# rcallahan/smalt

Hardware: AMD Instinct MI355X
Metric: mapped reads/sec (1Mx150bp vs 3Gbp ref) (higher is better)
Workload: dtype f16

## Files before the change

include/smaltgpu.h:

```cpp
#ifndef SMALTGPU_H
#define SMALTGPU_H
#include <stddef.h>
#include <stdint.h>

#ifdef __cplusplus
extern "C" {
#endif

enum {
  SMALTGPU_OK = 0,
  SMALTGPU_ENODEV = -1,
  SMALTGPU_EFILE = -2,
  SMALTGPU_EARG = -3,
  SMALTGPU_ENOMEM = -4,
  SMALTGPU_ECAP = -5,
  SMALTGPU_EINTERNAL = -6,
  SMALTGPU_ESCORE = -8,
  SMALTGPU_ECPLX = -9
};
#define SMALTGPU_IS_READ_ERROR(rv) ((rv) == SMALTGPU_ECAP || (rv) == SMALTGPU_EINTERNAL || (rv) == SMALTGPU_ESCORE || (rv) == SMALTGPU_ECPLX)

enum {
  SMALTGPU_FLG_CMPLXW = 0x01,
  SMALTGPU_FLG_BEST = 0x02,
// ... 239 lines not shown
typedef struct smaltgpu_inshist smaltgpu_inshist;
int smaltgpu_sample_interval(uint64_t npairs, int every);
int smaltgpu_inshist_from_sample(smaltgpu_inshist **out, const int32_t *sample, uint64_t n);
int smaltgpu_inshist_read(smaltgpu_inshist **out, const char *path);
void smaltgpu_inshist_free(smaltgpu_inshist *h);
enum { SMALTGPU_HIST_SAMPLED = 0, SMALTGPU_HIST_SMOOTHED = 1, SMALTGPU_HIST_SECTION = 2 };
int smaltgpu_inshist_text(smaltgpu_inshist *h, int what, int width, const char **text, uint64_t *len);
int smaltgpu_inshist_bounds(const smaltgpu_inshist *h, int32_t *lo, int32_t *hi, int32_t *nbins, uint64_t *total);
int smaltgpu_inshist_count(const smaltgpu_inshist *h, int32_t insert_size, int smoothed, int32_t *count, int32_t *cumulative);
int smaltgpu_report_set_inshist(smaltgpu_report *rp, const smaltgpu_inshist *h);
int smaltgpu_report_pair_inserts(const smaltgpu_report *rp, const int32_t **insert_size, const uint8_t **known, uint32_t *npairs);

int smaltgpu_index_seqnames(const smaltgpu_index *ix, const char *const **names, const uint64_t **sop, int64_t *nseq);

int smaltgpu_timers(const smaltgpu_mapper *m, double *ms, uint64_t *work, int n);
const char *smaltgpu_timer_name(int i);

int smaltgpu_set_debug(smaltgpu_mapper *m, int level);
long smaltgpu_dump_read(smaltgpu_mapper *m, uint32_t i, const char *name, char *buf, size_t bufsiz);

int smaltgpu_sw_full_batch(smaltgpu_mapper *m, const uint8_t *qcodes, const uint32_t *q_off, const uint8_t *rcodes,
                           const uint32_t *r_off, uint32_t ntask, const smaltgpu_params *par, int32_t *scores, int packed16);

int smaltgpu_rank_sort_batch(smaltgpu_mapper *m, const uint32_t *keys, const uint32_t *off, uint32_t narr, int nneed, int in_lds,
                             uint32_t *out_keys, uint32_t *out_idx);

const char *smaltgpu_last_error(void);
int smaltgpu_device_count(void);

#ifdef __cplusplus
}
#endif
#endif
```

smalt_amd/api.py:

```python
from __future__ import annotations

import ctypes as C
import os
from typing import List, Optional, Sequence

HERE = os.path.dirname(os.path.abspath(__file__))
LIBPATH = os.path.join(HERE, "libsmaltgpu.so")

FLG_CMPLXW, FLG_BEST, FLG_SEQBYSEQ, FLG_NOSHRTINFO, FLG_SENSITIVE = 0x01, 0x02, 0x10, 0x20, 0x80
ECAP, EINTERNAL, ESCORE, ECPLX = -5, -6, -8, -9


class SmaltGpuError(RuntimeError):
    def __init__(self, code, msg):
        super().__init__("smaltgpu error %d: %s" % (code, msg))
        self.code = code


class IndexDesc(C.Structure):
    _fields_ = [("k", C.c_int32), ("s", C.c_int32), ("typ", C.c_int32), ("nbits_key", C.c_int32), ("nbits_lo", C.c_int32),
                ("npos", C.c_uint32), ("nwords", C.c_uint32), ("idx", C.c_void_p), ("pos", C.c_void_p),
                ("wordidx", C.c_void_p), ("posidx", C.c_void_p), ("nseq", C.c_int64), ("sop", C.c_void_p),
                ("packed", C.c_void_p), ("on_device", C.c_int32)]

# ... 137 lines not shown
        L.smaltgpu_report_emit.argtypes = [C.c_void_p, C.POINTER(PostOut), C.POINTER(BatchOut), C.POINTER(ReadsView), C.POINTER(C.c_char_p), C.c_int64,
                                           C.POINTER(ReportOpts), C.c_int, C.POINTER(C.c_void_p), C.POINTER(C.c_uint64)]
        L.smaltgpu_pairs_create.restype = C.c_void_p
        L.smaltgpu_pairs_free.argtypes = [C.c_void_p]
        L.smaltgpu_map_pairs.argtypes = [C.c_void_p, C.c_void_p, C.c_void_p, C.c_void_p, C.c_void_p, C.c_void_p, C.c_void_p, C.c_uint32, C.POINTER(Params),
                                         C.POINTER(PairOpts), C.c_void_p]
        L.smaltgpu_pairs_timers.argtypes = [C.c_void_p, C.POINTER(C.c_double), C.POINTER(C.c_uint64)]
        L.smaltgpu_map_pairs_resident.argtypes = [C.c_void_p, C.POINTER(ResidentReads), C.c_void_p, C.c_void_p, C.c_void_p, C.c_void_p, C.c_uint32, C.POINTER(Params),
                                                  C.POINTER(PairOpts), C.c_void_p]
        L.smaltgpu_pairs_info.argtypes = [C.c_void_p, C.POINTER(C.c_uint32), C.POINTER(C.POINTER(PairInfo)), C.POINTER(C.c_uint64), C.POINTER(C.c_double)]
        L.smaltgpu_report_emit_pairs.argtypes = [C.c_void_p, C.c_void_p, C.POINTER(ReadsView), C.POINTER(ReadsView), C.POINTER(C.c_char_p), C.c_int64,
                                                 C.POINTER(ReportOpts), C.POINTER(PairOpts), C.c_int, C.POINTER(C.c_void_p), C.POINTER(C.c_uint64)]
        L.smaltgpu_index_seqnames.argtypes = [C.c_void_p, C.POINTER(C.POINTER(C.c_char_p)), C.POINTER(C.POINTER(C.c_uint64)), C.POINTER(C.c_int64)]
        L.smaltgpu_map_batch_device.argtypes = [C.c_void_p, C.c_void_p, C.c_void_p, C.c_void_p, C.c_uint32, C.c_uint64,
                                                C.POINTER(Params)]
        L.smaltgpu_fetch_results.argtypes = [C.c_void_p, C.POINTER(BatchOut)]
        L.smaltgpu_synchronize.argtypes = [C.c_void_p]
        L.smaltgpu_timers.argtypes = [C.c_void_p, C.POINTER(C.c_double), C.POINTER(C.c_uint64), C.c_int]
        L.smaltgpu_set_debug.argtypes = [C.c_void_p, C.c_int]
        L.smaltgpu_dump_read.restype = C.c_long
        L.smaltgpu_dump_read.argtypes = [C.c_void_p, C.c_uint32, C.c_char_p, C.c_char_p, C.c_size_t]
        L.smaltgpu_sw_full_batch.argtypes = [C.c_void_p, C.c_char_p, C.POINTER(C.c_uint32), C.c_char_p,
                                             C.POINTER(C.c_uint32), C.c_uint32, C.POINTER(Params), C.POINTER(C.c_int32), C.c_int]
        L.smaltgpu_rank_sort_batch.argtypes = [C.c_void_p, C.c_void_p, C.c_void_p, C.c_uint32, C.c_int, C.c_int, C.c_void_p, C.c_void_p]
        L.smaltgpu_sample_interval.argtypes = [C.c_uint64, C.c_int]
        L.smaltgpu_inshist_from_sample.argtypes = [C.POINTER(C.c_void_p), C.POINTER(C.c_int32), C.c_uint64]
        L.smaltgpu_inshist_read.argtypes = [C.POINTER(C.c_void_p), C.c_char_p]
        L.smaltgpu_inshist_free.argtypes = [C.c_void_p]
        L.smaltgpu_inshist_text.argtypes = [C.c_void_p, C.c_int, C.c_int, C.POINTER(C.c_void_p), C.POINTER(C.c_uint64)]
        L.smaltgpu_inshist_bounds.argtypes = [C.c_void_p, C.POINTER(C.c_int32), C.POINTER(C.c_int32), C.POINTER(C.c_int32), C.POINTER(C.c_uint64)]
        L.smaltgpu_inshist_count.argtypes = [C.c_void_p, C.c_int32, C.c_int, C.POINTER(C.c_int32), C.POINTER(C.c_int32)]
        L.smaltgpu_report_set_inshist.argtypes = [C.c_void_p, C.c_void_p]
        L.smaltgpu_report_pair_inserts.argtypes = [C.c_void_p, C.POINTER(C.POINTER(C.c_int32)), C.POINTER(C.POINTER(C.c_uint8)), C.POINTER(C.c_uint32)]
        _lib = L
    return _lib


def _check(rv):
    if rv != 0:
        raise SmaltGpuError(rv, lib().smaltgpu_last_error().decode())


def device_count() -> int:
    return lib().smaltgpu_device_count()


# ... 334 lines not shown
```

smalt_amd/csrc/smaltgpu.cpp:

```cpp
#include <hip/hip_runtime.h>
#include <math.h>
#include <stdarg.h>
#include <stdio.h>
#include <stdlib.h>
#include <string.h>
#include <mutex>
#include <string>
#include <thread>
#include <vector>
#include "../../include/smaltgpu.h"
#include "smg_dump.hpp"
#include "smg_indexfile.hpp"
#include "smg_indexbuild.h"
#include "smg_fasta.hpp"
#include "smg_kernels.h"

using namespace smg;

static thread_local std::string g_err;
static int fail(int code, const char *fmt, ...) {
  char buf[512];
  va_list ap;
  va_start(ap, fmt);
  vsnprintf(buf, sizeof(buf), fmt, ap);
// ... 1192 lines not shown
  uint32_t qmaxlen = 0;
  for (uint32_t t = 0; t < ntask; t++) { uint32_t l = q_off[t + 1] - q_off[t]; if (l > qmaxlen) qmaxlen = l; }
  int rv = 0;
  if (dalloc(&dq, q_off[ntask] + 16) || dalloc(&dr, r_off[ntask] + 16) || dalloc(&dqo, (size_t)ntask + 1) || dalloc(&dro, (size_t)ntask + 1) || dalloc(&dsc, ntask)) rv = SMALTGPU_ENOMEM;
  if (!rv) {
    (void)hipMemcpy(dq, qcodes, q_off[ntask], hipMemcpyHostToDevice);
    (void)hipMemcpy(dr, rcodes, r_off[ntask], hipMemcpyHostToDevice);
    (void)hipMemcpy(dqo, q_off, ((size_t)ntask + 1) * 4, hipMemcpyHostToDevice);
    (void)hipMemcpy(dro, r_off, ((size_t)ntask + 1) * 4, hipMemcpyHostToDevice);
    uint32_t rmaxlen = 0;
    for (uint32_t t = 0; t < ntask; t++) { uint32_t l = r_off[t + 1] - r_off[t]; if (l > rmaxlen) rmaxlen = l; }
    int lr;
    if (!packed16 && (qmaxlen > 512 || rmaxlen > (uint32_t)SW_FULL_WMAX))
      lr = launch_sw_strip_raw(m->stream, dq, dqo, dr, dro, ntask, to_par(par), dsc, m->strip_bnd, m->strip_win, m->wincap, m->strip_grid);
    else lr = launch_sw_full_raw(m->stream, dq, dqo, dr, dro, ntask, to_par(par), dsc, qmaxlen, packed16);
    if (lr) rv = fail(SMALTGPU_EARG, lr == -2 ? "scores do not fit the packed 16-bit kernel" : "query longer than the register-tiled kernel supports");
    else if (hipStreamSynchronize(m->stream) != hipSuccess) rv = fail(SMALTGPU_ENODEV, "kernel failed");
    else (void)hipMemcpy(scores, dsc, (size_t)ntask * 4, hipMemcpyDeviceToHost);
  }
  (void)hipFree(dq); (void)hipFree(dr); (void)hipFree(dqo); (void)hipFree(dro); (void)hipFree(dsc);
  return rv;
}

extern "C" int smaltgpu_rank_sort_batch(smaltgpu_mapper *m, const uint32_t *keys, const uint32_t *off, uint32_t narr, int nneed, int in_lds,
                                         uint32_t *out_keys, uint32_t *out_idx) {
  if (!m || !keys || !off || !out_keys || !out_idx) return fail(SMALTGPU_EARG, "null argument");
  HIPCHK(hipSetDevice(m->device));
  const size_t tot = off[narr];
  for (uint32_t t = 0; t < narr; t++) if (off[t + 1] < off[t] || off[t + 1] - off[t] > (1u << 22)) return fail(SMALTGPU_EARG, "bad array offsets");
  for (size_t i = 0; i < tot; i++) if (keys[i] >= 1024u) return fail(SMALTGPU_EARG, "key out of range");
  uint32_t *dk = nullptr, *doff = nullptr, *dkv = nullptr, *dok = nullptr, *doi = nullptr;
  int rv = 0;
  if (dalloc(&dk, tot + 1) || dalloc(&doff, (size_t)narr + 1) || dalloc(&dkv, tot + 1) || dalloc(&dok, tot + 1) || dalloc(&doi, tot + 1)) rv = SMALTGPU_ENOMEM;
  if (!rv) {
    (void)hipMemcpy(dk, keys, tot * 4, hipMemcpyHostToDevice);
    (void)hipMemcpy(doff, off, ((size_t)narr + 1) * 4, hipMemcpyHostToDevice);
    launch_rank_sort_raw(m->stream, dk, doff, narr, nneed, in_lds, dkv, dok, doi);
    if (hipStreamSynchronize(m->stream) != hipSuccess) rv = fail(SMALTGPU_ENODEV, "kernel failed");
    else { (void)hipMemcpy(out_keys, dok, tot * 4, hipMemcpyDeviceToHost); (void)hipMemcpy(out_idx, doi, tot * 4, hipMemcpyDeviceToHost); }
  }
  (void)hipFree(dk); (void)hipFree(doff); (void)hipFree(dkv); (void)hipFree(dok); (void)hipFree(doi);
  return rv;
}
```

smalt_amd/csrc/smg_kernels.h:

```cpp
#pragma once
#include <hip/hip_runtime_api.h>
#include "smg_cands.hpp"

namespace smg {

enum : int { SW_FULL_WMAX = 1016,
             SW_SHORT_WMAX = 248 };

int launch_encode(hipStream_t s, const uint8_t *bases, const uint64_t *off, uint32_t n, uint8_t *codes, uint8_t *codes_rc);
int launch_gather_reads(hipStream_t s, uint8_t *dst_bases, uint8_t *dst_quals, const uint64_t *dst_off, uint32_t n, const uint32_t *ids,
                        const uint8_t *const src_bases[2], const uint8_t *const src_quals[2], const uint64_t *const src_off[2]);
int launch_fine_index(hipStream_t s, const Batch &b, const DevIndex &ix);
int launch_seed(hipStream_t s, const Batch &b, const DevIndex &ix, const MapPar &p, uint8_t *scratch, size_t sbytes, uint32_t nslots);
struct CandGeom {
  uint32_t hcap;
  uint32_t hcap_strand;
  uint32_t ngrp, segcap, candcap;
  size_t slot_bytes;
  int debug;
  uint32_t window;
  uint32_t lds_hits, tab;
  int pass;
};
inline size_t cand_slot_bytes(const CandGeom &g, uint32_t qmax, int s) {
  size_t a = cand_scratch_bytes(qmax, s, g.hcap, g.ngrp, g.segcap, g.candcap);
  size_t b = cands_v2_hbm_bytes(qmax, s, g.hcap_strand, g.ngrp, g.candcap, true);
  return a > b ? a : b;
}
int launch_hits(hipStream_t s, const Batch &b, const DevIndex &ix, const MapPar &p, uint32_t W, uint32_t tab, uint32_t nwg);
int launch_cands(hipStream_t s, const Batch &b, const DevIndex &ix, const MapPar &p, uint8_t *scratch, uint32_t nslots, const CandGeom &g);
int launch_replay(hipStream_t s, const Batch &b, const DevIndex &ix, const MapPar &p);
int launch_align(hipStream_t s, const Batch &b, const DevIndex &ix, const MapPar &p, uint8_t *scratch, size_t sbytes, uint32_t nslots,
                 uint32_t wincap, uint64_t dircap, uint32_t rescap, uint32_t dstrcap, int pass, const CplxPar *cplx = nullptr);
int sw_full_geometry(uint32_t qmax_len, int *G, int *C);
int launch_sw_full(hipStream_t s, const Batch &b, const DevIndex &ix, const MapPar &p, uint32_t qmax_len, uint32_t ntask_cap, uint32_t grid);
int launch_sw_strip(hipStream_t s, const Batch &b, const DevIndex &ix, const MapPar &p, void *bnd, uint8_t *win, uint32_t wcap, uint32_t grid);
int launch_sw_strip_raw(hipStream_t s, const uint8_t *q, const uint32_t *qo, const uint8_t *r, const uint32_t *ro, uint32_t n, const MapPar &p,
                        int32_t *sc, void *bnd, uint8_t *win, uint32_t wcap, uint32_t grid);
int launch_sw_scalar(hipStream_t s, const Batch &b, const DevIndex &ix, const MapPar &p, int *rows, uint32_t rowlen, uint32_t nthreads,
                     uint32_t qmax_len);
int launch_sw_full_raw(hipStream_t s, const uint8_t *q, const uint32_t *qo, const uint8_t *r, const uint32_t *ro, uint32_t n,
                       const MapPar &p, int32_t *sc, uint32_t qmax_len, int packed16);
int launch_rank_sort_raw(hipStream_t s, const uint32_t *keys, const uint32_t *off, uint32_t narr, int nneed, int in_lds, uint32_t *kv,
                         uint32_t *out_key, uint32_t *out_idx);

}
```

smalt_amd/csrc/smg_kernels.hip:

```cpp
#include <hip/hip_runtime.h>
#include <cstdlib>
#include "smg_kernels.h"
#include "smg_stages.hpp"

namespace smg {

__device__ inline uint8_t code_of(uint8_t c) {
  c &= 0xDF;
  return c == 'A' ? 0 : c == 'C' ? 1 : c == 'G' ? 2 : (c == 'T' || c == 'U') ? 3 : 5;
}

__global__ void __launch_bounds__(64) k_encode(const uint8_t *bases, const uint64_t *off, uint32_t n, uint8_t *codes, uint8_t *codes_rc) {
  for (uint32_t r = blockIdx.x; r < n; r += gridDim.x) {
    const uint64_t o = off[r];
    const uint32_t len = (uint32_t)(off[r + 1] - o);
    for (uint32_t i = threadIdx.x; i < len; i += 64) {
      uint8_t c = code_of(bases[o + i]);
      codes[o + i] = c;
      codes_rc[o + len - 1 - i] = (c & 4) ? c : (uint8_t)(3 - c);
    }
  }
}

__global__ void __launch_bounds__(64) k_gather_reads(uint8_t *dst_bases, uint8_t *dst_quals, const uint64_t *dst_off, uint32_t n, const uint32_t *ids,
// ... 276 lines not shown
      cells += (unsigned long long)qlen * wlen;
      ntasks_done += best < 65535 ? 1 : 0;
    }
    __syncthreads();
  }
  for (int o = 32; o > 0; o >>= 1) { cells += __shfl_xor(cells, o); ntasks_done += __shfl_xor(ntasks_done, o); }
  if (lane == 0 && cells) { atomicAdd(b.work + WK_CELLS_FULL, cells); atomicAdd(b.work + WK_TASKS_FULL, ntasks_done); }
}

typedef unsigned short us2 __attribute__((ext_vector_type(2)));
__device__ inline us2 as_us2(uint32_t v) { return __builtin_bit_cast(us2, v); }
__device__ inline uint32_t as_u32(us2 v) { return __builtin_bit_cast(uint32_t, v); }
__device__ inline us2 pk_max(us2 a, us2 b) { return __builtin_elementwise_max(a, b); }
__device__ inline us2 pk_subs(us2 a, us2 b) { return __builtin_elementwise_sub_sat(a, b); }
__device__ inline us2 pk_add_nc(us2 a, us2 b) { return as_us2(as_u32(a) + as_u32(b)); }
typedef _Float16 hf2 __attribute__((ext_vector_type(2)));
__device__ inline us2 pk_max3(us2 a, us2 b, us2 c) {
  const hf2 r = __builtin_elementwise_maximum(__builtin_elementwise_maximum(__builtin_bit_cast(hf2, a), __builtin_bit_cast(hf2, b)), __builtin_bit_cast(hf2, c));
  return __builtin_bit_cast(us2, r);
}
__device__ inline uint32_t shr1_u32(uint32_t v) { return (uint32_t)__builtin_amdgcn_update_dpp(0, (int)v, 0x111 , 0xf, 0xf, true); }

enum : int { SW16_BLK = 5 };
struct Sw16Par { uint32_t mm4, dlt, n4; us2 bias, gi, ge; int fp; uint32_t hi_match, hi_mismatch; us2 ngi, nge; };
__device__ inline uint32_t f16_bits_of_int(int n) {
  if (n == 0) return 0;
  const uint32_t sign = n < 0 ? 0x8000u : 0u, a = (uint32_t)(n < 0 ? -n : n);
  const int e = 31 - __clz((int)a);
  return sign | ((uint32_t)(e + 15) << 10) | ((e <= 10 ? a << (10 - e) : a >> (e - 10)) & 0x3ffu);
}
__device__ inline Sw16Par sw16_par(const MapPar &p, int ncols = 512) {
  Sw16Par s;
  const uint32_t fm = f16_bits_of_int(p.match), fx = f16_bits_of_int(p.mismatch);
  s.fp = (fm & 0xffu) == 0 && (fx & 0xffu) == 0 && p.match > 0 && p.match * ncols <= 2040 && -p.gap_init >= 0 && -p.gap_init <= 2040 &&
         -p.gap_ext >= 0 && -p.gap_ext <= 2040 && p.mismatch >= -1024;
  s.hi_match = fm >> 8; s.hi_mismatch = fx >> 8;
  { const uint32_t a = f16_bits_of_int(p.gap_init), e = f16_bits_of_int(p.gap_ext);
    s.ngi = us2{(unsigned short)a, (unsigned short)a}; s.nge = us2{(unsigned short)e, (unsigned short)e}; }
  const int bias = (p.mismatch < p.mismatch - p.match ? -p.mismatch : -(p.mismatch - p.match));
  s.mm4 = (uint32_t)((p.mismatch + bias) & 0xff) * 0x01010101u;
  s.dlt = (uint32_t)(p.match - p.mismatch);
  s.n4 = (uint32_t)(bias & 0xff) * 0x01010101u;
  s.bias = us2{(unsigned short)bias, (unsigned short)bias};
  s.gi = us2{(unsigned short)(-p.gap_init), (unsigned short)(-p.gap_init)};
  s.ge = us2{(unsigned short)(-p.gap_ext), (unsigned short)(-p.gap_ext)};
  return s;
}

template <int G, int C>
__device__ inline uint32_t sw16_core(const uint16_t *wrow, int nstep, const uint32_t (&sel)[C], int g, const Sw16Par &sp, const uint2 *rowtab2) {
  us2 H[C], E[C];
#pragma unroll
  for (int cc = 0; cc < C; cc++) { H[cc] = us2{0, 0}; E[cc] = us2{0, 0}; }
  us2 best = us2{0, 0}, F = us2{0, 0}, prev_hl = us2{0, 0};
  const uint32_t gmask = g == 0 ? 0u : 0xffffffffu;
  for (int step = 0; step < nstep; step++) {
    const uint2 rr = rowtab2[wrow[step - g + (G - 1)]];
    const uint32_t rowA = rr.x, rowB = rr.y;
    const uint32_t hl = shr1_u32(as_u32(H[C - 1])) & gmask;
    const uint32_t fin = shr1_u32(as_u32(F)) & gmask;
    us2 carry = prev_hl;
// ... 72 lines not shown
        const int cc = c0 + u;
        if (cc < C) {
          const hf2 hh = hf_max3(t3[u], E[cc], F);
          H[cc] = hh;
          const hf2 tt = hh + ngi;
          E[cc] = hf_max3(E[cc] + nge, tt, zero);
          F = hf_max3(F + nge, tt, zero);
        }
      }
#pragma unroll
      for (int u = 0; u < SW16_BLK; u += 2) {
        const int cc = c0 + u;
        if (cc + 1 < C && u + 1 < SW16_BLK) best = hf_max3(best, H[cc], H[cc + 1]);
        else if (cc < C) best = __builtin_elementwise_maximum(best, H[cc]);
      }
      carry = last_old;
    }
  }
  for (int o = G / 2; o > 0; o >>= 1)
    best = __builtin_elementwise_maximum(best, __builtin_bit_cast(hf2, (uint32_t)__shfl_xor((int)__builtin_bit_cast(uint32_t, best), o)));
  return (uint32_t)(int)(float)best.x | ((uint32_t)(int)(float)best.y << 16);
}

__device__ inline void sw16_rowtab(uint32_t *rowtab, const Sw16Par &sp) {
  if (threadIdx.x < 8) rowtab[threadIdx.x] = threadIdx.x < 4 ? sp.mm4 + (sp.dlt << (8 * threadIdx.x)) : sp.n4;
}
__device__ inline void sw16_rowtab2(uint2 *rowtab2, const Sw16Par &sp) {
  const uint32_t a = threadIdx.x & 7u, bq = threadIdx.x >> 3;
  if (sp.fp) {
    const uint32_t x4 = sp.hi_mismatch * 0x01010101u;
    rowtab2[threadIdx.x] = make_uint2(a < 4 ? (x4 & ~(0xffu << (8 * a))) | (sp.hi_match << (8 * a)) : 0u,
                                      bq < 4 ? (x4 & ~(0xffu << (8 * bq))) | (sp.hi_match << (8 * bq)) : 0u);
    return;
  }
  rowtab2[threadIdx.x] = make_uint2(a < 4 ? sp.mm4 + (sp.dlt << (8 * a)) : sp.n4, bq < 4 ? sp.mm4 + (sp.dlt << (8 * bq)) : sp.n4);
}
enum : uint32_t { SW16_NPAIR = 5u | (5u << 3) };

template <int G, int C>
struct Sw16Geo {
  enum : int { CP = (C + 3) & ~3,
               NW = CP / 4, QST = G * CP };
};
typedef uint32_t __attribute__((may_alias)) u32_alias;
enum : uint32_t { SW16_PAD4 = 0x0c0c0c0cu, SW16_N10 = 0x2DB6DB6Du  };
constexpr int sw16_went(int G, int WMAX) { return (WMAX + 2 * G - 2 + 9) / 10 * 10; }

template <int G, int C, bool RAW>
__device__ inline bool sw16_stage(uint8_t *qst, const uint8_t *fw, const uint8_t *rc, uint32_t qlen) {
  constexpr uint32_t CP = Sw16Geo<G, C>::CP, QST = Sw16Geo<G, C>::QST;
  bool bad = false;
  for (uint32_t t = threadIdx.x; t < QST; t += 64) {
    const uint32_t gg = t / CP, cc = t % CP, j = gg * (uint32_t)C + cc;
    uint32_t a = 0x0cu, r = 0x0cu;
    if (cc < (uint32_t)C && j < qlen) {
      a = fw[j];
      if (RAW) { bad = bad || (a & 7u) >= 4u; a &= 3u; r = a; }
      else r = rc[j];
// ... 63 lines not shown
                                   const uint32_t (&ws)[2], const uint32_t (&wlen)[2]) {
  u32_alias *dst = (u32_alias *)wrow;
  const uint32_t nchunk = (nent + 9u) / 10u;
  uint32_t mlo[2], mhi[2];
#pragma unroll
  for (int u = 0; u < 2; u++) {
    const int64_t room = lastw - wbase[u];
    mlo[u] = wbase[u] < 0 ? (uint32_t)(-wbase[u]) : 0u;
    mhi[u] = room > 0x7fffffff ? 0x7fffffffu : (uint32_t)room;
  }
  for (uint32_t m = (uint32_t)g; m < nchunk; m += G) {
    const uint32_t ma = sw16_codes10<G>(packed, wbase[0], ws[0], m, mlo[0], mhi[0], wlen[0]);
    const uint32_t mb = sw16_codes10<G>(packed, wbase[1], ws[1], m, mlo[1], mhi[1], wlen[1]);
#pragma unroll
    for (int pr = 0; pr < 5; pr++) {
      const int s0 = 3 * (9 - 2 * pr), s1 = s0 - 3;
      const uint32_t e0 = ((ma >> s0) & 7u) | (((mb >> s0) & 7u) << 3), e1 = ((ma >> s1) & 7u) | (((mb >> s1) & 7u) << 3);
      dst[5 * m + (uint32_t)pr] = e0 | (e1 << 16);
    }
  }
}

template <int G, int C, int WMAX>
__global__ void __launch_bounds__(64) k_sw_full16(Batch b, DevIndex ix, MapPar p, uint32_t ntask_cap) {
  const unsigned long long nlong = WMAX > SW_SHORT_WMAX ? b.work[WK_LONG_TASKS] : 0;
  if (WMAX > SW_SHORT_WMAX && nlong == 0) return;
  const uint32_t *list = (WMAX > SW_SHORT_WMAX && b.long_list && nlong <= b.long_cap) ? b.long_list : nullptr;
  constexpr int NG = 64 / G, NW = Sw16Geo<G, C>::NW;
  __shared__ __attribute__((aligned(16))) uint16_t win[NG][sw16_went(G, WMAX)];
  __shared__ uint2 rowtab2[64];
  __shared__ __attribute__((aligned(16))) uint8_t qst[2 * Sw16Geo<G, C>::QST];
  const int lane = threadIdx.x, g = lane % G, grp = lane / G;
  const uint32_t ntask = list ? (uint32_t)nlong : min(*b.rc_count, ntask_cap), npair = (ntask + 1) / 2;
  const Sw16Par sp = sw16_par(p, G * C);
  sw16_rowtab2(rowtab2, sp);
  const uint32_t niter = (npair + NG - 1) / NG;
  const bool small = ix.totlen <= 0xffffffffull;
  const int64_t lastw = (int64_t)(ix.totlen / 10);
  uint32_t staged = 0xffffffffu;
  unsigned long long cells = 0, ntasks_done = 0;
  for (uint32_t it = blockIdx.x; it < niter; it += gridDim.x) {
    const uint32_t tp = it * NG + grp;
    uint32_t tix = 0, flags = 0, rid = 0, meta = 0, wlo = 0, whi = 0;
    {
      const uint32_t tl = 2 * tp + (uint32_t)g;
      if (g < 2 && tp < npair && tl < ntask) {
        tix = list ? list[tl] : tl;
        const RCand *rc = b.rcpool + tix;
        flags = rc->flags;
        const uint32_t r = rc->rid;
        const uint64_t rs = rc->rs;
        const uint32_t ql = read_len(b, r), wl = (uint32_t)(rc->re - rs + 1);
        if (!(flags & (RCF_BANDED | RCF_ERR | RCF_QN | RCF_SCORED)) && wl <= (uint32_t)WMAX && ql <= (uint32_t)(G * C)) {
          const int32_t sq = rc->sqidx;
          int64_t wb; uint32_t s;
          sw16_win_origin<G>((sq < 0 ? 0ull : ix.sop[sq]) + rs, small, wb, s);
          rid = r; wlo = (uint32_t)(uint64_t)wb; whi = (uint32_t)((uint64_t)wb >> 32);
          meta = ql | (wl << 10) | (s << 20) | ((flags & RCF_REVERSE) ? 1u << 24 : 0u) | (1u << 25);
// ... 17 lines not shown
    nstep = __builtin_amdgcn_readfirstlane(nstep);
    sw16_window<G>(win[grp], g, (uint32_t)(nstep + G - 1), ix.packed, lastw, wbase, ws, wlen);
    uint32_t xa[NW], xb[NW];
#pragma unroll
    for (int w = 0; w < NW; w++) { xa[w] = SW16_PAD4; xb[w] = SW16_PAD4; }
    bool pend0 = live[0], pend1 = live[1];
    for (;;) {
      const unsigned long long pm = __ballot(pend0 || pend1);
      if (!pm) break;
      const uint32_t R = (uint32_t)__builtin_amdgcn_readlane((int)(pend0 ? key[0] : key[1]), __ffsll(pm) - 1);
      if (R != staged) {
        __syncthreads();
        const uint64_t o = b.read_off[R];
        sw16_stage<G, C, false>(qst, b.codes + o, b.codes_rc + o, (uint32_t)(b.read_off[R + 1] - o));
        staged = R;
        __syncthreads();
      }
      if (pend0 && key[0] == R) { sw16_fetch<G, C>(xa, qst, g, rev[0]); pend0 = false; }
      if (pend1 && key[1] == R) { sw16_fetch<G, C>(xb, qst, g, rev[1]); pend1 = false; }
    }
    uint32_t sel[C];
    sw16_sel<G, C>(sel, xa, xb, sp.fp);
    __syncthreads();
    const uint32_t bb = sp.fp ? sw16f_core<G, C>(win[grp], nstep, sel, g, sp, rowtab2) : sw16_core<G, C>(win[grp], nstep, sel, g, sp, rowtab2);
    if ((meta >> 25) & 1u) {
      const int best = (int)((bb >> (16 * g)) & 0xffffu);
      b.rcpool[tix].swscor = best;
      b.rcpool[tix].flags = flags | RCF_SCORED | (best >= 65535 ? RCF_BANDED : 0u);
      cells += (unsigned long long)(meta & 0x3ffu) * ((meta >> 10) & 0x3ffu);
      ntasks_done += best < 65535 ? 1 : 0;
    }
    __syncthreads();
  }
  for (int o = 32; o > 0; o >>= 1) { cells += __shfl_xor(cells, o); ntasks_done += __shfl_xor(ntasks_done, o); }
  if (lane == 0 && cells) { atomicAdd(b.work + WK_CELLS_FULL, cells); atomicAdd(b.work + WK_TASKS_FULL, ntasks_done); }
}

template <int G, int C>
__global__ void __launch_bounds__(64) k_sw_full16_raw(const uint8_t *qcodes, const uint32_t *q_off, const uint8_t *rcodes,
                                                       const uint32_t *r_off, uint32_t ntask, MapPar p, int32_t *scores) {
  constexpr int NG = 64 / G, NW = Sw16Geo<G, C>::NW;
  constexpr int WMAX = SW_FULL_WMAX;
  __shared__ uint16_t win[NG][WMAX + 2 * G];
  __shared__ uint2 rowtab2[64];
  __shared__ __attribute__((aligned(16))) uint8_t qst[2 * Sw16Geo<G, C>::QST];
  const int lane = threadIdx.x, g = lane % G, grp = lane / G;
  const uint32_t npair = (ntask + 1) / 2;
  const Sw16Par sp = sw16_par(p, G * C);
  sw16_rowtab2(rowtab2, sp);
  const uint32_t ngroups = gridDim.x * NG;
  for (uint32_t t0 = blockIdx.x * NG; t0 < npair; t0 += ngroups) {
    const uint32_t tp = t0 + grp;
    bool live[2] = {false, false};
    uint32_t qlen[2] = {0, 0}, wlen[2] = {0, 0}, key[2] = {0, 0};
    const uint8_t *r[2] = {rcodes, rcodes};
#pragma unroll
    for (int u = 0; u < 2; u++) {
      const uint32_t t = 2 * tp + (uint32_t)u;
      if (tp < npair && t < ntask) {
        qlen[u] = q_off[t + 1] - q_off[t]; wlen[u] = r_off[t + 1] - r_off[t];
        r[u] += r_off[t]; key[u] = t;
        live[u] = wlen[u] <= (uint32_t)WMAX && qlen[u] <= (uint32_t)(G * C);
      }
      if (!live[u]) { qlen[u] = 0; wlen[u] = 0; }
    }
    const uint32_t wmax = wlen[0] > wlen[1] ? wlen[0] : wlen[1];
    int nstep = (int)wmax + G - 1;
    for (int o = 32; o > 0; o >>= 1) nstep = max(nstep, __shfl_xor(nstep, o));
    nstep = __builtin_amdgcn_readfirstlane(nstep);
    for (uint32_t e = g; e < (uint32_t)(nstep + G - 1); e += G) {
      const uint32_t i = e - (uint32_t)(G - 1);
      uint32_t cd[2];
#pragma unroll
      for (int u = 0; u < 2; u++) { const uint32_t x = i < wlen[u] ? (r[u][i] & 7u) : 5u; cd[u] = x == 7 ? 0 : ((x == 6 || x == 4) ? 5 : x); }
      win[grp][e] = (uint16_t)(cd[0] | (cd[1] << 3));
    }
    uint32_t xa[NW], xb[NW];
#pragma unroll
    for (int w = 0; w < NW; w++) { xa[w] = SW16_PAD4; xb[w] = SW16_PAD4; }
    bool qn[2] = {false, false};
    bool pend0 = live[0], pend1 = live[1];
    for (;;) {
      const unsigned long long pm = __ballot(pend0 || pend1);
      if (!pm) break;
      const uint32_t R = (uint32_t)__builtin_amdgcn_readlane((int)(pend0 ? key[0] : key[1]), __ffsll(pm) - 1);
      __syncthreads();
      const uint32_t o = q_off[R];
      const bool bad = sw16_stage<G, C, true>(qst, qcodes + o, qcodes + o, q_off[R + 1] - o);
      __syncthreads();
      if (pend0 && key[0] == R) { sw16_fetch<G, C>(xa, qst, g, false); qn[0] = bad; pend0 = false; }
      if (pend1 && key[1] == R) { sw16_fetch<G, C>(xb, qst, g, false); qn[1] = bad; pend1 = false; }
    }
    uint32_t sel[C];
    sw16_sel<G, C>(sel, xa, xb, sp.fp);
    __syncthreads();
    const uint32_t bb = sp.fp ? sw16f_core<G, C>(win[grp], nstep, sel, g, sp, rowtab2) : sw16_core<G, C>(win[grp], nstep, sel, g, sp, rowtab2);
    if (g == 0) {
#pragma unroll
      for (int u = 0; u < 2; u++) {
        const uint32_t t = 2 * tp + (uint32_t)u;
        if (tp < npair && t < ntask) scores[t] = !live[u] ? -1 : (qn[u] ? -2 : (int)((bb >> (16 * u)) & 0xffffu));
      }
    }
    __syncthreads();
  }
}

enum : int { SW_STRIP_C = 16 };

__device__ inline int sw_strip_core(const uint8_t *q, uint32_t qlen, const uint8_t *win, uint32_t wlen, int2 *bnd, uint32_t wcap,
                                    const uint2 *tab, int2 *ring , int bias, int gi, int ge) {
  constexpr int C = SW_STRIP_C;
  const int g = (int)threadIdx.x;
  int2 *ring_in = ring, *ring_out = ring + 128;
  int best = 0;
  const uint32_t nstrip = (qlen + 64 * C - 1) / (64 * C);
  const int nstep = (int)wlen + 63;
  for (uint32_t sidx = 0; sidx < nstrip; sidx++) {
    const int2 *bprev = bnd + (size_t)((sidx + 1) & 1) * wcap;
// ... 587 lines not shown
  } else if (b.qmax > 256) hipLaunchKernelGGL((k_align<true, false>), dim3(grid), dim3(64), dyn, s, b, ix, p, scratch, sbytes, wincap, dircap, rescap, dstrcap, lds_bytes, pass, NoCplx());
  else hipLaunchKernelGGL((k_align<false, false>), dim3(grid), dim3(64), dyn, s, b, ix, p, scratch, sbytes, wincap, dircap, rescap, dstrcap, lds_bytes, pass, NoCplx());
  SMG_LAUNCH_CHECK();
  return 0;
}

int sw_full_geometry(uint32_t qmax_len, int *G, int *C) {
  if (qmax_len <= 64) { *G = 4; *C = 16; }
  else if (qmax_len <= 104) { *G = 8; *C = 13; }
  else if (qmax_len <= 152) { *G = 8; *C = 19; }
  else if (qmax_len <= 160) { *G = 8; *C = 20; }
  else if (qmax_len <= 256) { *G = 16; *C = 16; }
  else if (qmax_len <= 512) { *G = 16; *C = 32; }
  else { *G = 0; *C = 0; return -1; }
  return 0;
}

static bool sw16_ok(const MapPar &p) {
  const int bias = (p.mismatch < p.mismatch - p.match ? -p.mismatch : -(p.mismatch - p.match));
  return p.match > 0 && p.match * 512 + bias + 256 < 0x7C00  && bias >= 0 && p.match + bias < 256 && p.mismatch + bias >= 0 &&
         -p.gap_init >= 0 && -p.gap_init < 30000 && -p.gap_ext >= 0 && -p.gap_ext < 30000;
}

template <int G, int C>
static void launch_sw_full_t(hipStream_t s, const Batch &b, const DevIndex &ix, const MapPar &p, uint32_t ntask_cap, uint32_t grid) {
  const int use16 = sw16_ok(p);
  if (use16) {
    hipLaunchKernelGGL((k_sw_full16<G, C, SW_SHORT_WMAX>), dim3(grid), dim3(64), 0, s, b, ix, p, ntask_cap);
    hipLaunchKernelGGL((k_sw_full16<G, C, SW_FULL_WMAX>), dim3(grid), dim3(64), 0, s, b, ix, p, ntask_cap);
  }
  hipLaunchKernelGGL((k_sw_full<G, C>), dim3(grid), dim3(64), 0, s, b, ix, p, ntask_cap, use16);
}

int launch_sw_full(hipStream_t s, const Batch &b, const DevIndex &ix, const MapPar &p, uint32_t qmax_len, uint32_t ntask_cap, uint32_t grid) {
  int G, C;
  if (sw_full_geometry(qmax_len, &G, &C)) return 0;
  if (G == 4) launch_sw_full_t<4, 16>(s, b, ix, p, ntask_cap, grid);
  else if (G == 8 && C == 13) launch_sw_full_t<8, 13>(s, b, ix, p, ntask_cap, grid);
  else if (G == 8 && C == 19) launch_sw_full_t<8, 19>(s, b, ix, p, ntask_cap, grid);
  else if (G == 8) launch_sw_full_t<8, 20>(s, b, ix, p, ntask_cap, grid);
  else if (C == 16) launch_sw_full_t<16, 16>(s, b, ix, p, ntask_cap, grid);
  else launch_sw_full_t<16, 32>(s, b, ix, p, ntask_cap, grid);
  SMG_LAUNCH_CHECK();
  return 0;
}

int launch_sw_strip(hipStream_t s, const Batch &b, const DevIndex &ix, const MapPar &p, void *bnd, uint8_t *win, uint32_t wcap, uint32_t grid) {
  if (!b.nreads || !grid) return 0;
  if (sw16_ok(p) && (uint64_t)b.qmax * (uint64_t)p.match < 60000ull)
  {
    if ((uint64_t)b.qmax * (uint64_t)p.match + 512 < 0x7C00ull)
      hipLaunchKernelGGL(k_sw_strip16<true>, dim3(grid), dim3(64), 0, s, b, ix, p, (uint2 *)bnd, (uint16_t *)win, wcap);
// ... 5 lines not shown
  return 0;
}

int launch_sw_strip_raw(hipStream_t s, const uint8_t *q, const uint32_t *qo, const uint8_t *r, const uint32_t *ro, uint32_t n, const MapPar &p,
                        int32_t *sc, void *bnd, uint8_t *win, uint32_t wcap, uint32_t grid) {
  if (!n) return 0;
  hipLaunchKernelGGL(k_sw_strip_raw, dim3(n < grid ? n : grid), dim3(64), 0, s, q, qo, r, ro, n, p, sc, (int2 *)bnd, win, wcap);
  SMG_LAUNCH_CHECK();
  return 0;
}

int launch_sw_scalar(hipStream_t s, const Batch &b, const DevIndex &ix, const MapPar &p, int *rows, uint32_t rowlen, uint32_t nthreads,
                     uint32_t qmax_len) {
  int G, C;
  int full_gc = sw_full_geometry(qmax_len, &G, &C) ? 0 : G * C;
  hipLaunchKernelGGL(k_sw_scalar, dim3(nthreads / 64), dim3(64), 0, s, b, ix, p, rows, rowlen, full_gc);
  SMG_LAUNCH_CHECK();
  return 0;
}

template <int G, int C>
static void launch_sw_raw_t(hipStream_t s, const uint8_t *q, const uint32_t *qo, const uint8_t *r, const uint32_t *ro, uint32_t n,
                            const MapPar &p, int32_t *sc, uint32_t grid, int packed16) {
  if (packed16) hipLaunchKernelGGL((k_sw_full16_raw<G, C>), dim3(grid), dim3(64), 0, s, q, qo, r, ro, n, p, sc);
  else hipLaunchKernelGGL((k_sw_full_raw<G, C>), dim3(grid), dim3(64), 0, s, q, qo, r, ro, n, p, sc);
}

__global__ void __launch_bounds__(64) k_rank_sort_raw(const uint32_t *keys, const uint32_t *off, uint32_t narr, int nneed, int in_lds,
                                                      uint32_t *kv, uint32_t *out_key, uint32_t *out_idx) {
  __shared__ uint32_t sh[16 + WSORT_WORDS + 8192];
  uint32_t *wk = sh + 16, *arr = wk + WSORT_WORDS;
  for (uint32_t t = blockIdx.x; t < narr; t += gridDim.x) {
    const uint32_t o = off[t], n = off[t + 1] - o;
    uint32_t *a = (in_lds && n <= 8192) ? arr : kv + o;
    for (uint32_t i = threadIdx.x; i < n; i += 64) a[i] = (keys[o + i] << WSORT_IDXBITS) | i;
    __syncthreads();
    wave_sort_kv(a, (int)n, nneed < 0 ? (int)n : nneed, wk);
    __syncthreads();
    for (uint32_t i = threadIdx.x; i < n; i += 64) { out_key[o + i] = a[i] >> WSORT_IDXBITS; out_idx[o + i] = a[i] & ((1u << WSORT_IDXBITS) - 1u); }
    __syncthreads();
  }
}

int launch_rank_sort_raw(hipStream_t s, const uint32_t *keys, const uint32_t *off, uint32_t narr, int nneed, int in_lds, uint32_t *kv,
                         uint32_t *out_key, uint32_t *out_idx) {
  if (!narr) return 0;
  hipLaunchKernelGGL(k_rank_sort_raw, dim3(narr < 4096 ? narr : 4096), dim3(64), 0, s, keys, off, narr, nneed, in_lds, kv, out_key, out_idx);
// ... 24 lines not shown
```

Measured before the change: 789,400.

## Add row-relative frame f16 Smith-Waterman core for short windows

Adds an alternative fp16 SW inner loop that keeps scores in a per-row shifted reference frame: gap extension is folded into the substitution table and the running offset is subtracted at the end. Per-step floor clamps drop out and a max3 replaces separate max/add operations. The new core is used only when the step count is small enough that fp16 stays exact for the given scoring parameters; otherwise the existing cores run. It adds a second LDS row table and an environment switch, and relies on a host/device bound check holding exactly, since f16 rounding could otherwise corrupt scores.

```diff
diff --git a/include/smaltgpu.h b/include/smaltgpu.h
--- a/include/smaltgpu.h
+++ b/include/smaltgpu.h
@@ -285,6 +285,8 @@
 int smaltgpu_sw_full_batch(smaltgpu_mapper *m, const uint8_t *qcodes, const uint32_t *q_off, const uint8_t *rcodes,
                            const uint32_t *r_off, uint32_t ntask, const smaltgpu_params *par, int32_t *scores, int packed16);
 
+int smaltgpu_sw_rowframe_max_steps(int match, int mismatch, int gap_init, int gap_ext, int ncols);
+
 int smaltgpu_rank_sort_batch(smaltgpu_mapper *m, const uint32_t *keys, const uint32_t *off, uint32_t narr, int nneed, int in_lds,
                              uint32_t *out_keys, uint32_t *out_idx);
 
diff --git a/smalt_amd/api.py b/smalt_amd/api.py
--- a/smalt_amd/api.py
+++ b/smalt_amd/api.py
@@ -183,6 +183,7 @@
         L.smaltgpu_dump_read.argtypes = [C.c_void_p, C.c_uint32, C.c_char_p, C.c_char_p, C.c_size_t]
         L.smaltgpu_sw_full_batch.argtypes = [C.c_void_p, C.c_char_p, C.POINTER(C.c_uint32), C.c_char_p,
                                              C.POINTER(C.c_uint32), C.c_uint32, C.POINTER(Params), C.POINTER(C.c_int32), C.c_int]
+        L.smaltgpu_sw_rowframe_max_steps.argtypes = [C.c_int] * 5
         L.smaltgpu_rank_sort_batch.argtypes = [C.c_void_p, C.c_void_p, C.c_void_p, C.c_uint32, C.c_int, C.c_int, C.c_void_p, C.c_void_p]
         L.smaltgpu_sample_interval.argtypes = [C.c_uint64, C.c_int]
         L.smaltgpu_inshist_from_sample.argtypes = [C.POINTER(C.c_void_p), C.POINTER(C.c_int32), C.c_uint64]
diff --git a/smalt_amd/csrc/smaltgpu.cpp b/smalt_amd/csrc/smaltgpu.cpp
--- a/smalt_amd/csrc/smaltgpu.cpp
+++ b/smalt_amd/csrc/smaltgpu.cpp
@@ -1238,6 +1238,10 @@
   return rv;
 }
 
+extern "C" int smaltgpu_sw_rowframe_max_steps(int match, int mismatch, int gap_init, int gap_ext, int ncols) {
+  return sw16_rowframe_max_steps(match, mismatch, gap_init, gap_ext, ncols);
+}
+
 extern "C" int smaltgpu_rank_sort_batch(smaltgpu_mapper *m, const uint32_t *keys, const uint32_t *off, uint32_t narr, int nneed, int in_lds,
                                          uint32_t *out_keys, uint32_t *out_idx) {
   if (!m || !keys || !off || !out_keys || !out_idx) return fail(SMALTGPU_EARG, "null argument");
diff --git a/smalt_amd/csrc/smg_kernels.h b/smalt_amd/csrc/smg_kernels.h
--- a/smalt_amd/csrc/smg_kernels.h
+++ b/smalt_amd/csrc/smg_kernels.h
@@ -41,6 +41,7 @@
                      uint32_t qmax_len);
 int launch_sw_full_raw(hipStream_t s, const uint8_t *q, const uint32_t *qo, const uint8_t *r, const uint32_t *ro, uint32_t n,
                        const MapPar &p, int32_t *sc, uint32_t qmax_len, int packed16);
+int sw16_rowframe_max_steps(int match, int mismatch, int gap_init, int gap_ext, int ncols);
 int launch_rank_sort_raw(hipStream_t s, const uint32_t *keys, const uint32_t *off, uint32_t narr, int nneed, int in_lds, uint32_t *kv,
                          uint32_t *out_key, uint32_t *out_idx);
 
diff --git a/smalt_amd/csrc/smg_kernels.hip b/smalt_amd/csrc/smg_kernels.hip
--- a/smalt_amd/csrc/smg_kernels.hip
+++ b/smalt_amd/csrc/smg_kernels.hip
@@ -322,12 +322,27 @@
 __device__ inline uint32_t shr1_u32(uint32_t v) { return (uint32_t)__builtin_amdgcn_update_dpp(0, (int)v, 0x111 , 0xf, 0xf, true); }
 
 enum : int { SW16_BLK = 5 };
-struct Sw16Par { uint32_t mm4, dlt, n4; us2 bias, gi, ge; int fp; uint32_t hi_match, hi_mismatch; us2 ngi, nge; };
+struct Sw16Par { uint32_t mm4, dlt, n4; us2 bias, gi, ge; int fp; uint32_t hi_match, hi_mismatch; us2 ngi, nge;
+                 int rf_steps; uint32_t hi_rmatch, hi_rmismatch, hi_rn; us2 pge, ngo; };
 __device__ inline uint32_t f16_bits_of_int(int n) {
   if (n == 0) return 0;
   const uint32_t sign = n < 0 ? 0x8000u : 0u, a = (uint32_t)(n < 0 ? -n : n);
   const int e = 31 - __clz((int)a);
   return sign | ((uint32_t)(e + 15) << 10) | ((e <= 10 ? a << (10 - e) : a >> (e - 10)) & 0x3ffu);
+}
+__host__ __device__ inline int sw16_rowframe_steps(int match, int mismatch, int gap_init, int gap_ext, int ncols) {
+  const int gi = -gap_init, ge = -gap_ext;
+  if (match <= 0 || ge < 0 || gi < ge || gi > 2040 || mismatch < -1024 || match + ge > 2040) return -1;
+  const int sc[5] = {match + ge, mismatch + ge, ge, match, mismatch};
+  for (int k = 0; k < 5; k++) {
+    int a = sc[k] < 0 ? -sc[k] : sc[k];
+    while (a && !(a & 1)) a >>= 1;
+    if (a > 7) return -1;
+  }
+  const int room = 2040 - gi - match * ncols;
+  if (room < 0) return -1;
+  if (ge == 0) return 0x7fffffff;
+  return room / ge - 1;
 }
 __device__ inline Sw16Par sw16_par(const MapPar &p, int ncols = 512) {
   Sw16Par s;
@@ -337,6 +352,11 @@
   s.hi_match = fm >> 8; s.hi_mismatch = fx >> 8;
   { const uint32_t a = f16_bits_of_int(p.gap_init), e = f16_bits_of_int(p.gap_ext);
     s.ngi = us2{(unsigned short)a, (unsigned short)a}; s.nge = us2{(unsigned short)e, (unsigned short)e}; }
+  s.rf_steps = s.fp ? sw16_rowframe_steps(p.match, p.mismatch, p.gap_init, p.gap_ext, ncols) : -1;
+  s.hi_rmatch = f16_bits_of_int(p.match - p.gap_ext) >> 8; s.hi_rmismatch = f16_bits_of_int(p.mismatch - p.gap_ext) >> 8;
+  s.hi_rn = f16_bits_of_int(-p.gap_ext) >> 8;
+  { const uint32_t e = f16_bits_of_int(-p.gap_ext), o = f16_bits_of_int(p.gap_init - p.gap_ext);
+    s.pge = us2{(unsigned short)e, (unsigned short)e}; s.ngo = us2{(unsigned short)o, (unsigned short)o}; }
   const int bias = (p.mismatch < p.mismatch - p.match ? -p.mismatch : -(p.mismatch - p.match));
   s.mm4 = (uint32_t)((p.mismatch + bias) & 0xff) * 0x01010101u;
   s.dlt = (uint32_t)(p.match - p.mismatch);
@@ -455,6 +475,65 @@
   return (uint32_t)(int)(float)best.x | ((uint32_t)(int)(float)best.y << 16);
 }
 
+template <int G, int C>
+__device__ inline uint32_t sw16r_core(const uint16_t *wrow, int nstep, const uint32_t (&sel)[C], int g, const Sw16Par &sp, const uint2 *rowtab2r) {
+  hf2 H[C], E[C];
+  const hf2 pge = __builtin_bit_cast(hf2, sp.pge), nge = __builtin_bit_cast(hf2, sp.nge), ngo = __builtin_bit_cast(hf2, sp.ngo);
+  const _Float16 r0 = (_Float16)(-(g + 1));
+  hf2 flo1 = pge * hf2{r0, r0} + pge;
+  {
+    const hf2 f0 = flo1 - pge;
+#pragma unroll
+    for (int cc = 0; cc < C; cc++) { H[cc] = f0; E[cc] = flo1; }
+  }
+  hf2 best = flo1 - pge, F = best, prev_hl = best, flo = best;
+  const uint32_t gmask = g == 0 ? 0u : 0xffffffffu;
+  for (int step = 0; step < nstep; step++) {
+    const uint2 rr = rowtab2r[wrow[step - g + (G - 1)]];
+    flo = flo1;
+    flo1 = flo + pge;
+    const uint32_t flob = __builtin_bit_cast(uint32_t, flo);
+    const uint32_t hl = (shr1_u32(__builtin_bit_cast(uint32_t, H[C - 1])) & gmask) | (flob & ~gmask);
+    const uint32_t fin = (shr1_u32(__builtin_bit_cast(uint32_t, F)) & gmask) | (flob & ~gmask);
+    hf2 carry = prev_hl;
+    prev_hl = __builtin_bit_cast(hf2, hl);
+    F = __builtin_bit_cast(hf2, fin);
+#define SW16R_SB() __builtin_amdgcn_sched_barrier(0)
+    hf2 t3[C + 2];
+    t3[0] = carry + __builtin_bit_cast(hf2, __builtin_amdgcn_perm(rr.y, rr.x, sel[0]));
+    if (C > 1) t3[1] = H[0] + __builtin_bit_cast(hf2, __builtin_amdgcn_perm(rr.y, rr.x, sel[1]));
+    SW16R_SB();
+#pragma unroll
+    for (int cc = 0; cc < C; cc++) {
+      const hf2 hh = hf_max3(t3[cc], E[cc], F);
+      SW16R_SB();
+      hf2 w = hh;
+      if (cc + 2 < C) w = __builtin_bit_cast(hf2, __builtin_amdgcn_perm(rr.y, rr.x, sel[cc + 2 < C ? cc + 2 : 0]));
+      SW16R_SB();
+      const hf2 tt = hh + ngo;
+      SW16R_SB();
+      if (cc + 2 < C) t3[cc + 2] = H[cc + 1 < C ? cc + 1 : 0] + w;
+      SW16R_SB();
+      const hf2 fm = __builtin_elementwise_maximum(F, tt);
+      SW16R_SB();
+      E[cc] = hf_max3(E[cc], tt, flo1);
+      H[cc] = hh;
+      SW16R_SB();
+      F = fm + nge;
+      SW16R_SB();
+      if (cc & 1) best = hf_max3(best, H[cc - 1], H[cc]);
+      else if (cc == 0) best = best + pge;
+      else if (cc == C - 1) best = __builtin_elementwise_maximum(best, H[cc]);
+      SW16R_SB();
+    }
+#undef SW16R_SB
+  }
+  best = best - flo;
+  for (int o = G / 2; o > 0; o >>= 1)
+    best = __builtin_elementwise_maximum(best, __builtin_bit_cast(hf2, (uint32_t)__shfl_xor((int)__builtin_bit_cast(uint32_t, best), o)));
+  return (uint32_t)(int)(float)best.x | ((uint32_t)(int)(float)best.y << 16);
+}
+
 __device__ inline void sw16_rowtab(uint32_t *rowtab, const Sw16Par &sp) {
   if (threadIdx.x < 8) rowtab[threadIdx.x] = threadIdx.x < 4 ? sp.mm4 + (sp.dlt << (8 * threadIdx.x)) : sp.n4;
 }
@@ -467,6 +546,12 @@
     return;
   }
   rowtab2[threadIdx.x] = make_uint2(a < 4 ? sp.mm4 + (sp.dlt << (8 * a)) : sp.n4, bq < 4 ? sp.mm4 + (sp.dlt << (8 * bq)) : sp.n4);
+}
+__device__ inline void sw16_rowtab2r(uint2 *rowtab2r, const Sw16Par &sp) {
+  const uint32_t a = threadIdx.x & 7u, bq = threadIdx.x >> 3;
+  const uint32_t x4 = sp.hi_rmismatch * 0x01010101u, n4 = sp.hi_rn * 0x01010101u;
+  rowtab2r[threadIdx.x] = make_uint2(a < 4 ? (x4 & ~(0xffu << (8 * a))) | (sp.hi_rmatch << (8 * a)) : n4,
+                                     bq < 4 ? (x4 & ~(0xffu << (8 * bq))) | (sp.hi_rmatch << (8 * bq)) : n4);
 }
 enum : uint32_t { SW16_NPAIR = 5u | (5u << 3) };
 
@@ -576,18 +661,20 @@
 }
 
 template <int G, int C, int WMAX>
-__global__ void __launch_bounds__(64) k_sw_full16(Batch b, DevIndex ix, MapPar p, uint32_t ntask_cap) {
+__global__ void __launch_bounds__(64) k_sw_full16(Batch b, DevIndex ix, MapPar p, uint32_t ntask_cap, int rowframe) {
   const unsigned long long nlong = WMAX > SW_SHORT_WMAX ? b.work[WK_LONG_TASKS] : 0;
   if (WMAX > SW_SHORT_WMAX && nlong == 0) return;
   const uint32_t *list = (WMAX > SW_SHORT_WMAX && b.long_list && nlong <= b.long_cap) ? b.long_list : nullptr;
   constexpr int NG = 64 / G, NW = Sw16Geo<G, C>::NW;
   __shared__ __attribute__((aligned(16))) uint16_t win[NG][sw16_went(G, WMAX)];
-  __shared__ uint2 rowtab2[64];
+  __shared__ uint2 rowtab2[64], rowtab2r[64];
   __shared__ __attribute__((aligned(16))) uint8_t qst[2 * Sw16Geo<G, C>::QST];
   const int lane = threadIdx.x, g = lane % G, grp = lane / G;
   const uint32_t ntask = list ? (uint32_t)nlong : min(*b.rc_count, ntask_cap), npair = (ntask + 1) / 2;
   const Sw16Par sp = sw16_par(p, G * C);
   sw16_rowtab2(rowtab2, sp);
+  const int rf_steps = rowframe ? sp.rf_steps : -1;
+  if (rf_steps >= 0) sw16_rowtab2r(rowtab2r, sp);
   const uint32_t niter = (npair + NG - 1) / NG;
   const bool small = ix.totlen <= 0xffffffffull;
   const int64_t lastw = (int64_t)(ix.totlen / 10);
@@ -651,7 +738,8 @@
     uint32_t sel[C];
     sw16_sel<G, C>(sel, xa, xb, sp.fp);
     __syncthreads();
-    const uint32_t bb = sp.fp ? sw16f_core<G, C>(win[grp], nstep, sel, g, sp, rowtab2) : sw16_core<G, C>(win[grp], nstep, sel, g, sp, rowtab2);
+    const uint32_t bb = nstep <= rf_steps ? sw16r_core<G, C>(win[grp], nstep, sel, g, sp, rowtab2r)
+                        : sp.fp ? sw16f_core<G, C>(win[grp], nstep, sel, g, sp, rowtab2) : sw16_core<G, C>(win[grp], nstep, sel, g, sp, rowtab2);
     if ((meta >> 25) & 1u) {
       const int best = (int)((bb >> (16 * g)) & 0xffffu);
       b.rcpool[tix].swscor = best;
@@ -667,16 +755,18 @@
 
 template <int G, int C>
 __global__ void __launch_bounds__(64) k_sw_full16_raw(const uint8_t *qcodes, const uint32_t *q_off, const uint8_t *rcodes,
-                                                       const uint32_t *r_off, uint32_t ntask, MapPar p, int32_t *scores) {
+                                                       const uint32_t *r_off, uint32_t ntask, MapPar p, int32_t *scores, int rowframe) {
   constexpr int NG = 64 / G, NW = Sw16Geo<G, C>::NW;
   constexpr int WMAX = SW_FULL_WMAX;
   __shared__ uint16_t win[NG][WMAX + 2 * G];
-  __shared__ uint2 rowtab2[64];
+  __shared__ uint2 rowtab2[64], rowtab2r[64];
   __shared__ __attribute__((aligned(16))) uint8_t qst[2 * Sw16Geo<G, C>::QST];
   const int lane = threadIdx.x, g = lane % G, grp = lane / G;
   const uint32_t npair = (ntask + 1) / 2;
   const Sw16Par sp = sw16_par(p, G * C);
   sw16_rowtab2(rowtab2, sp);
+  const int rf_steps = rowframe ? sp.rf_steps : -1;
+  if (rf_steps >= 0) sw16_rowtab2r(rowtab2r, sp);
   const uint32_t ngroups = gridDim.x * NG;
   for (uint32_t t0 = blockIdx.x * NG; t0 < npair; t0 += ngroups) {
     const uint32_t tp = t0 + grp;
@@ -723,7 +813,8 @@
     uint32_t sel[C];
     sw16_sel<G, C>(sel, xa, xb, sp.fp);
     __syncthreads();
-    const uint32_t bb = sp.fp ? sw16f_core<G, C>(win[grp], nstep, sel, g, sp, rowtab2) : sw16_core<G, C>(win[grp], nstep, sel, g, sp, rowtab2);
+    const uint32_t bb = nstep <= rf_steps ? sw16r_core<G, C>(win[grp], nstep, sel, g, sp, rowtab2r)
+                        : sp.fp ? sw16f_core<G, C>(win[grp], nstep, sel, g, sp, rowtab2) : sw16_core<G, C>(win[grp], nstep, sel, g, sp, rowtab2);
     if (g == 0) {
 #pragma unroll
       for (int u = 0; u < 2; u++) {
@@ -1357,12 +1448,21 @@
          -p.gap_init >= 0 && -p.gap_init < 30000 && -p.gap_ext >= 0 && -p.gap_ext < 30000;
 }
 
+static int sw16_rowframe_on() {
+  const char *e = getenv("SMALTGPU_SW16_ROWFRAME");
+  return !(e && e[0] == '0');
+}
+int sw16_rowframe_max_steps(int match, int mismatch, int gap_init, int gap_ext, int ncols) {
+  return sw16_rowframe_steps(match, mismatch, gap_init, gap_ext, ncols);
+}
+
 template <int G, int C>
 static void launch_sw_full_t(hipStream_t s, const Batch &b, const DevIndex &ix, const MapPar &p, uint32_t ntask_cap, uint32_t grid) {
   const int use16 = sw16_ok(p);
   if (use16) {
-    hipLaunchKernelGGL((k_sw_full16<G, C, SW_SHORT_WMAX>), dim3(grid), dim3(64), 0, s, b, ix, p, ntask_cap);
-    hipLaunchKernelGGL((k_sw_full16<G, C, SW_FULL_WMAX>), dim3(grid), dim3(64), 0, s, b, ix, p, ntask_cap);
+    const int rf = sw16_rowframe_on();
+    hipLaunchKernelGGL((k_sw_full16<G, C, SW_SHORT_WMAX>), dim3(grid), dim3(64), 0, s, b, ix, p, ntask_cap, rf);
+    hipLaunchKernelGGL((k_sw_full16<G, C, SW_FULL_WMAX>), dim3(grid), dim3(64), 0, s, b, ix, p, ntask_cap, rf);
   }
   hipLaunchKernelGGL((k_sw_full<G, C>), dim3(grid), dim3(64), 0, s, b, ix, p, ntask_cap, use16);
 }
@@ -1414,7 +1514,7 @@
 template <int G, int C>
 static void launch_sw_raw_t(hipStream_t s, const uint8_t *q, const uint32_t *qo, const uint8_t *r, const uint32_t *ro, uint32_t n,
                             const MapPar &p, int32_t *sc, uint32_t grid, int packed16) {
-  if (packed16) hipLaunchKernelGGL((k_sw_full16_raw<G, C>), dim3(grid), dim3(64), 0, s, q, qo, r, ro, n, p, sc);
+  if (packed16) hipLaunchKernelGGL((k_sw_full16_raw<G, C>), dim3(grid), dim3(64), 0, s, q, qo, r, ro, n, p, sc, sw16_rowframe_on());
   else hipLaunchKernelGGL((k_sw_full_raw<G, C>), dim3(grid), dim3(64), 0, s, q, qo, r, ro, n, p, sc);
 }
 
```

After: 850,700 (median of 6 runs). +7.8%, better.
